# lmb-freiburg/optical-flow-2d-data-generation

Measured on AMD Instinct MI355X. Metric: training samples/sec (img0+img1+flow, 512x384), higher is better.
Workload: dtype u8 blends / fp64 affines -> f32 planes

## Files before the change

### optical-flow-2d-data-generation_amd/csrc/kernels.hip

```cpp
#include <hip/hip_runtime.h>
#include <stdint.h>
#include <type_traits>

#include "../../include/ofdg_detmath.h"
#include "ofdg_device.h"
#include "warpfields.h"

namespace ofdg {

__device__ __forceinline__ int iround_d(double v) {
  return (int)((v < 0.0) ? v - 0.5 : v + 0.5);
}
__device__ __forceinline__ void xform(const Mat& m, double& x, double& y) {
  double t = x;
  x = t * m.sx + y * m.shx + m.tx;
  y = t * m.shy + y * m.sy + m.ty;
}
__device__ __forceinline__ long long floordiv64(long long a, long long b) {
  long long q = (long long)floor((double)a / (double)b);
  long long r = a - q * b;
  if (r < 0) --q;
  else if (r >= b) ++q;
  return q;
}
// ... 497 lines not shown
  int nonzero = 0;
  for (int r = 0; r < rows; ++r) {
    const int2 cv = *reinterpret_cast<const int2*>(&tc.cover[r][c2]);
    const int2 ar = *reinterpret_cast<const int2*>(&tc.area[r][c2]);
    const int s2 = cv.x + cv.y;
    const int base = tc.carry[r] + wave_scan_incl(s2) - s2;
    int a0 = ((base + cv.x) << 9) - ar.x, a1 = ((base + s2) << 9) - ar.y;
    a0 >>= 9; a1 >>= 9;
    a0 = a0 < 0 ? -a0 : a0; a1 = a1 < 0 ? -a1 : a1;
    a0 = a0 > 255 ? 255 : a0; a1 = a1 > 255 ? 255 : a1;
    if (in_range) { *reinterpret_cast<uint16_t*>(dst + (size_t)r * W + c2) = (uint16_t)(a0 | (a1 << 8)); nonzero |= a0 | a1; }
  }
  const unsigned long long nz = __ballot(nonzero != 0);
  if (blockmask) {
    const int half = lane >> 5;
    if ((lane & 31) == 0 && ((nz >> (32 * half)) & 0xFFFFFFFFull)) {
      const int nbx = (W + kTileW - 1) / kTileW, nby = (H + kBandRows - 1) / kBandRows;
      atomicOr(blockmask + ((size_t)(sample * nby + band) * nbx + (X0 / kTileW + half)) * 2 + (sf & 1), 1ull << obj_local);
    }
  }
  __builtin_amdgcn_fence(__ATOMIC_ACQ_REL, "workgroup");
}

__global__ __launch_bounds__(64 * kRasterWaves) void raster_kernel(const DevShapeFrame* __restrict__ frames,
                                                     const int4* __restrict__ items,
                                                     const int* __restrict__ item_count,
                                                     const int2* __restrict__ verts, int W, int H,
                                                     uint8_t* __restrict__ cov,
                                                     unsigned long long* __restrict__ blockmask_next, int n_mask_words,
                                                     unsigned long long* __restrict__ blockmask) {
  __shared__ __attribute__((aligned(16))) RasterWs s_ws[kRasterWaves];
  step_kernel_priority();
  const int wave = threadIdx.x >> 6, lane = threadIdx.x & 63;
  for (int gid = blockIdx.x * blockDim.x + threadIdx.x; gid < n_mask_words; gid += gridDim.x * blockDim.x) blockmask_next[gid] = 0ull;
  const int n_items = *item_count;
  const int n_waves = gridDim.x * kRasterWaves;
  typedef OFDG_CONSTANT const int4 ConstItem;
  typedef OFDG_CONSTANT const DevShapeFrame ConstFrame;
  int it = __builtin_amdgcn_readfirstlane(blockIdx.x * kRasterWaves + wave);
  if (it >= n_items) return;
  struct Item { int sf, band, X0, X1; };
  struct Frame { int nv, x0, y0, x1, y1, sample, obj_local; };
  auto item_at = [&](int i) {
    const int4 q = ((ConstItem*)items)[i];
    return Item{q.x, q.y, q.z, q.w};
  };
  auto frame_of = [&](int sf) {
    const ConstFrame& f = ((ConstFrame*)frames)[sf];
    return Frame{f.n_verts, f.x0, f.y0, f.x1, f.y1, f.pad[0], f.pad[1]};
  };
  auto uni = [](int x) { return __builtin_amdgcn_readfirstlane(x); };
  int it1 = it + n_waves;
  Item I0 = item_at(it), I1 = item_at(it1 < n_items ? it1 : it);
  Frame F0 = frame_of(I0.sf);
  int2 pa = verts[(size_t)I0.sf * kMaxVerts + lane], pb = verts[(size_t)I0.sf * kMaxVerts + lane + 1];
  for (;;) {
    I0 = Item{uni(I0.sf), uni(I0.band), uni(I0.X0), uni(I0.X1)};
    I1 = Item{uni(I1.sf), uni(I1.band), uni(I1.X0), uni(I1.X1)};
    F0 = Frame{uni(F0.nv), uni(F0.x0), uni(F0.y0), uni(F0.x1), uni(F0.y1), uni(F0.sample), uni(F0.obj_local)};
    it1 = uni(it1);
    const int it2 = it1 + n_waves;
    const Item I2 = item_at(it2 < n_items ? it2 : it1 < n_items ? it1 : it);
    const Frame F1 = frame_of(I1.sf);
    const int2 na = verts[(size_t)I1.sf * kMaxVerts + lane], nb = verts[(size_t)I1.sf * kMaxVerts + lane + 1];
    raster_item(s_ws[wave], verts + (size_t)I0.sf * kMaxVerts, F0.nv, F0.x0, F0.y0, F0.x1, F0.y1, I0.sf, I0.band, I0.X0, I0.X1, W, H, cov, blockmask,
                F0.sample, F0.obj_local, lane, pa, pb);
    if (it1 >= n_items) break;
    I0 = I1; F0 = F1; I1 = I2; pa = na; pb = nb;
    it = it1; it1 = it2;
  }
}

__device__ __forceinline__ int aa_byte(int c) { return c == 255 ? 255 : (255 * c) >> 8; }
__device__ __forceinline__ int div255(int a) { return (a + 1 + (a >> 8)) >> 8; }
__device__ __forceinline__ int blend(int d, int s, int m) { return div255(m * s + (255 - m) * d); }

__device__ __forceinline__ uint32_t blend_px(uint32_t d, uint32_t s, uint32_t m) {
  const uint32_t im = 255u - m;
  uint32_t rb = m * (s & 0x00FF00FFu) + im * (d & 0x00FF00FFu);
  uint32_t g = m * ((s >> 8) & 255u) + im * ((d >> 8) & 255u);
  rb = ((rb + 0x00010001u + ((rb >> 8) & 0x00FF00FFu)) >> 8) & 0x00FF00FFu;
  g = (g + 1u + (g >> 8)) >> 8;
  return rb | (g << 8);
}

__device__ __forceinline__ float byte_over_255(int u) {
  const float fu = (float)u, c = 0x1.010102p-8f;
  const float q0 = __fmul_rn(fu, c);
  return __fmaf_rn(__fmaf_rn(-q0, 255.f, fu), c, q0);
}
__device__ __forceinline__ int comp_add(int u, int v) {
  const float fu = byte_over_255(u), fv = byte_over_255(v);
  const float t = __fmul_rn(__fsub_rn(1.f, fu), __fsub_rn(1.f, fv));
// ... 1257 lines not shown
#pragma unroll
    for (int c = 0; c < 3; ++c) {
      const double v1 = u32_to_double((t0 >> (8 * c)) & 255u), v2 = u32_to_double((t1 >> (8 * c)) & 255u);
      out |= (uint32_t)(unsigned char)(al1 * v1 + al * v2) << (8 * c);
    }
    return out;
  }
  if (sdim == n) return t0;
  const uint32_t d0 = u1, d1 = u2, d2 = (uint32_t)n - u1 - u2;
  uint32_t acc[3];
#pragma unroll
  for (int c = 0; c < 3; ++c)
    acc[c] = __umul24((t2 >> (8 * c)) & 255u, d2) + (__umul24((t1 >> (8 * c)) & 255u, d1) + __umul24((t0 >> (8 * c)) & 255u, d0));
  if (div24) return mulhi_u24(acc[0], mdiv) | (mulhi_u24(acc[1], mdiv) << 8) | (mulhi_u24(acc[2], mdiv) << 16);
  uint32_t out = 0;
#pragma unroll
  for (int c = 0; c < 3; ++c) {
    uint32_t q = __umulhi(acc[c], mdiv);
    q -= (q * (uint32_t)n > acc[c]) ? 1u : 0u;
    out |= q << (8 * c);
  }
  return out;
}
__global__ __launch_bounds__(64) void bgprep_stream_kernel(const DevBgPrep* __restrict__ prep, DevResizeTabs T, int W, int H, int n_samples,
                                                           int cap_cw, int cap_ch, uint32_t* __restrict__ B, uint32_t* __restrict__ err,
                                                           uint32_t* __restrict__ paths) {
  __shared__ uint32_t s_c[kPrepG][kPrepCW];
  extern __shared__ int s_first[];
  const int TW = 2 * W, TH = 2 * H, lane = threadIdx.x;
  {
    int running = 0;
    if (lane == 0) s_first[0] = 0;
    for (int c = 0; c < n_samples; c += 64) {
      const int i = c + lane;
      int nt = 0;
      if (i < n_samples) {
        const DevBgPrep& q = prep[i];
        const bool fits = prep_sample_fits(q, cap_cw, cap_ch);
        if (!fits && blockIdx.x == 0) atomicOr(err, kErrBgPrepCapacity);
        nt = fits ? prep_tile_cols(q) * prep_tile_rows(q) : 0;
      }
      const int incl = wave_scan_incl(nt);
      if (i < n_samples) s_first[i + 1] = running + incl;
      running += __shfl(incl, 63, 64);
    }
  }
  __syncthreads();
  const int total = __builtin_amdgcn_readfirstlane(s_first[n_samples]);
  auto sample_of = [&](int t) {
    int n = 0;
    for (int c = 0; c < n_samples; c += 64) {
      const int i = c + lane;
      n += __popcll(__ballot(i < n_samples && t >= s_first[i + 1]));
    }
    return __builtin_amdgcn_readfirstlane(n);
  };
  auto tab_index = [](int n, int dim, int k) { return (uint32_t)(n < dim ? n * dim + k : 0); };
  struct PrepBox { int cw, ch, rx0, ry0, rx1, ry1; };
  typedef OFDG_CONSTANT const DevBgPrep ConstPrep;
  auto box_fields = [&](int s) { const ConstPrep& q = ((ConstPrep*)prep)[s]; return PrepBox{q.cw, q.ch, q.rx0, q.ry0, q.rx1, q.ry1}; };
  auto box_of = [&](const PrepBox& q, int t, int s, PrepTile& F) {
    const int tcols = (q.rx1 - q.rx0 + kPrepW) / kPrepW;
    const int ti = t - __builtin_amdgcn_readfirstlane(s_first[s]), ty = ti / tcols, tx = ti - ty * tcols;
    F.s = s;
    F.bx0 = q.rx0 + tx * kPrepW; F.bx1 = min(F.bx0 + kPrepW - 1, q.rx1);
    F.by0 = q.ry0 + ty * kPrepH; F.by1 = min(F.by0 + kPrepH - 1, q.ry1);
  };
  int t = blockIdx.x;
  if (t < (int)(gridDim.x / (8 * kPrepRun)) * (8 * kPrepRun)) {
    const int xcd = t & 7, slot = t >> 3;
    t = ((slot / kPrepRun) * 8 + xcd) * kPrepRun + (slot % kPrepRun);
  }
  if (t >= total) return;
  PrepTile cur;
  int ex0, ex1, ey0, ey1;
  {
    const int s0 = sample_of(t);
    const PrepBox q = box_fields(s0);
    box_of(q, t, s0, cur);
    ex0 = tab_entry_uniform(T.at_x, tab_index(q.cw, TW, cur.bx0)); ex1 = tab_entry_uniform(T.at_x, tab_index(q.cw, TW, cur.bx1));
    ey0 = tab_entry_uniform(T.at_y, tab_index(q.ch, TH, cur.by0)); ey1 = tab_entry_uniform(T.at_y, tab_index(q.ch, TH, cur.by1));
  }
  for (;;) {
    const int tn = t + (int)gridDim.x;
    const bool more = tn < total;
    const int sc = __builtin_amdgcn_readfirstlane(cur.s);
    const int sn = more ? sample_of(tn) : sc;
    const DevBgPrep p = ((ConstPrep*)prep)[sc];
    const PrepBox qn = box_fields(sn);
    prep_finish_tile(p, cur, TW, TH, ex0, ex1, ey0, ey1);
    const int bx0 = cur.bx0, bx1 = cur.bx1, by0 = cur.by0, by1 = cur.by1;
    const int cx0 = cur.cx0, cx1 = cur.cx1, cy0 = cur.cy0, cy1 = cur.cy1;
    const int ncw = cx1 - cx0 + 1, nch = cy1 - cy0 + 1;
    const int x = bx0 + lane;
    const bool have_x = x <= bx1;
    const AxisEntry ex = axis_entry(p.cw, TW, min(x, bx1), T.at_x, T.alpha_x);
    const AxisEntry ey = axis_entry(p.ch, TH, min(by0 + lane, by1), T.at_y, T.alpha_y);
    PrepTile nxt = cur;
    int nx0 = 0, nx1 = 0, ny0 = 0, ny1 = 0;
    if (more) {
      box_of(qn, tn, sn, nxt);
      nx0 = tab_entry_uniform(T.at_x, tab_index(qn.cw, TW, nxt.bx0)); nx1 = tab_entry_uniform(T.at_x, tab_index(qn.cw, TW, nxt.bx1));
      ny0 = tab_entry_uniform(T.at_y, tab_index(qn.ch, TH, nxt.by0)); ny1 = tab_entry_uniform(T.at_y, tab_index(qn.ch, TH, nxt.by1));
    }
    if (!cur.fits) {
      if (lane == 0) atomicOr(err, kErrBgPrepCapacity);
    } else {
// ... 109 lines not shown
        } else {
        int xg = x, cwg = p.cw, chg = p.ch;
        asm volatile("" : "+v"(xg), "+s"(cwg), "+s"(chg));
        for (int r = 0; r < rows; ++r) {
          const int j = cy0 + g0 + r;
          m0 = m1; m1 = m2;
          m2 = have_x ? axis_texel(cwg, TW, xg, ex.u1, ex.u2, x_exact, s_c[r][xi0], s_c[r][xi1], s_c[r][xi2], xdiv, xdiv24, T.alpha_x) : 0u;
          emit_rows(j, [&](int dj, uint32_t v1, uint32_t v2) {
            uint32_t t0 = m2, t1 = m2;
            if (dj >= 2) { t0 = m0; t1 = m1; } else if (dj == 1) { t0 = m1; }
            return axis_texel(chg, TH, y, v1, v2, (v2 >> 31) != 0u, t0, t1, m2, ydiv, ydiv24, T.alpha_y);
          });
        }
        }
        __syncthreads();
      }
    }
    if (!more) break;
    ex0 = nx0; ex1 = nx1; ey0 = ny0; ey1 = ny1;
    cur = nxt;
    t = tn;
  }
}

__global__ __launch_bounds__(256) void bgprep_kernel(const DevBgPrep* __restrict__ prep, int W, int H, uint32_t* __restrict__ bgtex) {
  const int TW = 2 * W, TH = 2 * H, quads = TW / 4;
  const int s = blockIdx.y;
  const int i = blockIdx.x * blockDim.x + threadIdx.x;
  if (i >= quads * TH) return;
  const int v = i / quads, u0 = (i - v * quads) * 4;
  const DevBgPrep p = prep[s];
  if (v < p.ry0 || v > p.ry1 || u0 + 3 < p.rx0 || u0 > p.rx1) return;
  uint4 o;
  o.x = bgprep_texel(p, u0, v);
  o.y = bgprep_texel(p, u0 + 1, v);
  o.z = bgprep_texel(p, u0 + 2, v);
  o.w = bgprep_texel(p, u0 + 3, v);
  *reinterpret_cast<uint4*>(bgtex + (size_t)s * TW * TH + (size_t)v * TW + u0) = o;
}

__global__ __launch_bounds__(256) void pool_synth_kernel(uint32_t* __restrict__ pool, int n, int w, int h, uint32_t seed) {
  const size_t total = (size_t)n * w * h;
  for (size_t i = (size_t)blockIdx.x * blockDim.x + threadIdx.x; i < total; i += (size_t)gridDim.x * blockDim.x) {
    const uint32_t tex = (uint32_t)(i / ((size_t)w * h));
    const uint32_t rem = (uint32_t)(i - (size_t)tex * w * h);
    const uint32_t y = rem / w, x = rem - y * w;
// ... 115 lines not shown
```

### optical-flow-2d-data-generation_amd/csrc/ofdg_api.hip

```cpp
#include <hip/hip_runtime.h>
#include <hip/hip_ext.h>

#include <algorithm>
#include <cmath>
#include <cstdio>
#include <cstdlib>
#include <cstring>
#include <memory>
#include <string>
#include <vector>

#include "../../include/ofdg.h"
#include "kernels.hip"
#include "sampler_counter.hip"
#include "ofdg_device.h"
#include "realize.h"
#include "sampler_ref.h"
#include "warpfields.h"

using namespace ofdg;

static thread_local std::string g_create_error;
static const int g_hw_queues_env = [] { const char* q = std::getenv("GPU_MAX_HW_QUEUES"); return q ? std::atoi(q) : 0; }();

// ... 34 lines not shown
  std::vector<std::pair<int, int>> mixed_sizes;
  std::vector<uint32_t*> mixed_images;
  std::vector<DevTexEntry> tex_table;
  DevTexEntry* d_tex_table = nullptr;
  int pool_kind = OFDG_POOL_UNIFORM;
  uint32_t pool_seed = 0;
  std::unique_ptr<RefSampler> sampler;
  long long step = 0;
  struct Slot {
    RealizedBatch batch;
    DevBuf<DevShape> d_shapes;
    DevBuf<DevShapeFrame> d_frames;
    DevBuf<int2> d_verts;
    DevBuf<DevObject> d_objects;
    DevBuf<DevSample> d_samples;
    DevBuf<char> d_rec;
    DevBuf<int4> d_items;
    DevBuf<DevBgPrep> d_bgprep;
    DevBuf<uint32_t> d_bgtex;
    DevBuf<uint32_t> d_bgC;
    DevBuf<unsigned long long> d_blockmask;
    int res_objects = 0;
    bool bgprep_pending = false;
    int box_parity = 0;
    size_t box_stride = 0;
    int mask_used[2] = {0, 0};
    hipEvent_t ev_uploaded = nullptr;
    bool upload_pending = false;
    hipStream_t upload_stream = nullptr;
    DevBuf<DevCropRef> d_croptab;
    DevBuf<float> d_bgwarp;
    DevBuf<unsigned> d_bgwarp_max;
    hipEvent_t compose_event = nullptr;
    bool compose_pending = false;
    hipStream_t compose_stream = nullptr;
    int* d_item_count = nullptr;
    int res_samples = 0, res_shapes = 0;
  };
  static constexpr int kUserSlots = 16;
  Slot slots[kUserSlots];
  struct Stage {
    void* h = nullptr;
    size_t bytes = 0;
    hipEvent_t free_ev = nullptr;
    bool pending = false;
  };
// ... 673 lines not shown
  return OFDG_OK;
}
static void bgprep_caps(ofdg_ctx* c, int* cap_cw, int* cap_ch, bool* fusable) {
  if (c->bg_cap_n == c->pool_n && c->bg_cap_cw > 0) { *cap_cw = c->bg_cap_cw; *cap_ch = c->bg_cap_ch; *fusable = c->bg_fusable; return; }
  const int TW = 2 * c->prm.width, TH = 2 * c->prm.height;
  int cw = (int)((float)TW / 0.75f) + 2, ch = (int)((float)TH / 0.75f) + 2;
  bool all_large = true;
  auto small = [&](int w, int h) { if (w < TW || h < TH) { all_large = false; cw = std::max(cw, w + h / 8 + 4); ch = std::max(ch, h + w / 8 + 4); } };
  if (c->pool_mixed) for (const auto& wh : c->mixed_sizes) small(wh.first, wh.second);
  else small(c->pool_w, c->pool_h);
  c->bg_cap_cw = cw; c->bg_cap_ch = ch; c->bg_cap_n = c->pool_n; c->bg_fusable = all_large;
  *cap_cw = cw; *cap_ch = ch; *fusable = all_large;
}

static int reserve_workspaces(ofdg_ctx* c, size_t n_shapes) {
  const size_t need_cov = n_shapes * 2 * (size_t)c->prm.width * c->prm.height + 16;
  if (need_cov <= c->chains[0].cov.cap) return OFDG_OK;
  HIP_OK(c, hipDeviceSynchronize());
  for (int k = 0; k < c->n_chains; ++k) HIP_OK(c, c->chains[k].cov.reserve(need_cov));
  return OFDG_OK;
}

static int prepare_backgrounds(ofdg_ctx* c, ofdg_ctx::Slot& sl, int n, bool records_resident, hipStream_t s, uint32_t* err, hipEvent_t stop = nullptr);
static int launch_counter_sampler(ofdg_ctx* c, ofdg_ctx::Slot& sl, long long first_index, hipStream_t s, uint32_t* err) {
  const int stride = sl.res_shapes / sl.res_samples;
  const int prep = c->prm.background_prep ? 1 : 0;
  CsRealizeDims D{c->prm.width, c->prm.height, c->pool_n, c->pool_w, c->pool_h, sl.res_samples, stride, prep,
                  c->prm.mode == 9 ? c->crop_server.n_crops : 0, c->fg_src.stride, c->fg_src.origin, c->bg_src.stride, c->bg_src.origin,
                  (unsigned long long)(uintptr_t)c->pool, c->d_tex_table, c->prm.mode == 9 ? c->d_cs_croptab : nullptr};
  hipLaunchKernelGGL(cs_sample_realize_kernel, dim3(sl.res_samples * kCsGroups), dim3(64), 0, s, c->cs_mode, D, first_index,
                     sl.d_shapes.p, sl.d_objects.p, sl.d_samples.p, err, sl.d_bgprep.p);
  HIP_OK(c, hipGetLastError());
  sl.bgprep_pending = prep != 0;
  return OFDG_OK;
}

static void* own_stream(ofdg_ctx* c, void* stream) { return stream == OFDG_STREAM_OWN ? ofdg_stream(c) : stream; }

static ofdg_ctx::Chain& take_chain(ofdg_ctx* c) {
  const int k = (int)(c->next_chain % (unsigned)c->n_chains);
  c->next_chain++;
  c->last_chain = k;
  return c->chains[k];
}
static hipStream_t chain_stream(const ofdg_ctx* c, const ofdg_ctx::Chain& ch, hipStream_t st) { return c->overlap ? ch.stream : st; }

// ... 8 lines not shown
  return OFDG_OK;
}
static int discard_all_prepared(ofdg_ctx* c) {
  c->bg_cap_n = -1;
  for (int k = 0; k < c->n_chains; ++k) { int rc = discard_prepared(c, c->chains[k]); if (rc != OFDG_OK) return rc; }
  return OFDG_OK;
}

static RenderDims render_dims(const ofdg_ctx* c, const ofdg_ctx::Slot& sl) {
  const int W = c->prm.width, H = c->prm.height;
  RenderDims dm;
  dm.W = W; dm.H = H; dm.pool_w = c->pool_w; dm.pool_h = c->pool_h;
  dm.use_aa = c->prm.use_antialiasing ? 1 : 0;
  dm.n_samples = sl.res_samples;
  dm.n_shapes = sl.res_shapes;
  dm.tiles_x = (W + kTileW - 1) / kTileW;
  dm.tiles_y = (H + kTileH - 1) / kTileH;
  dm.bg_pitch = c->prm.background_prep ? 2 * W : c->bg_src.pitch;
  dm.fg_pitch = c->fg_src.pitch;
  return dm;
}

static int launch_prepare(ofdg_ctx* c, ofdg_ctx::Chain& ch, ofdg_ctx::Slot& sl, hipStream_t st, long long cs_first_index = -1,
                          bool hand_over = true) {
  const int W = c->prm.width, H = c->prm.height;
  const int n_sf = sl.res_shapes * 2;
  const RenderDims dm = render_dims(c, sl);
  { int rc = discard_prepared(c, ch); if (rc != OFDG_OK) return rc; }
  const long long ticket = c->ticket++;
  uint32_t* const err = err_word(c, ticket);
  hipEvent_t* ev = nullptr;
  if (c->profiling && c->ev_sets > 0 && (c->launch_count % c->ev_stride) == 0) {
    const size_t set = (size_t)(c->ev_alloc++ % c->ev_sets);
    ev = &c->ev[set * 6];
    c->ev_composed[set] = 0;
    c->ev_bgprep[set] = 0;
  }
  c->launch_count++;
  if (!c->overlap) {
    if (c->have_last_user_st && c->last_user_st != st) HIP_OK(c, hipDeviceSynchronize());
    c->last_user_st = st; c->have_last_user_st = true;
  }
  hipStream_t S = chain_stream(c, ch, st);
  uint8_t* cov = ch.cov.p;
  if (sl.upload_pending && sl.upload_stream != S) {
    if (hipEventQuery(sl.ev_uploaded) == hipSuccess) sl.upload_pending = false;
    else HIP_OK(c, hipStreamWaitEvent(S, sl.ev_uploaded, 0));
  }
  if (ch.done_pending && ch.done_stream != S) {
    if (hipEventQuery(ch.ev_done) != hipSuccess) HIP_OK(c, hipStreamWaitEvent(S, ch.ev_done, 0));
    ch.done_pending = false;
  }
  if (sl.compose_pending && sl.compose_stream != S) {
    if (hipEventQuery(sl.compose_event) == hipSuccess) sl.compose_pending = false;
    else HIP_OK(c, hipStreamWaitEvent(S, sl.compose_event, 0));
  }
  const DevCropRef* croptab = cs_first_index >= 0 ? c->d_cs_croptab : sl.d_croptab.p;
  HIP_OK(c, take_err_word(c, ticket, S));
  if (cs_first_index >= 0) {
    int rc = launch_counter_sampler(c, sl, cs_first_index, S, err);
    if (rc != OFDG_OK) return rc;
  }
  const int bp = sl.box_parity;
  sl.box_parity ^= 1;
  unsigned long long* box_cur = sl.d_blockmask.p + (size_t)bp * sl.box_stride;
  unsigned long long* box_next = sl.d_blockmask.p + (size_t)(bp ^ 1) * sl.box_stride;
  sl.mask_used[bp] = sl.res_samples * dm.tiles_x * ((H + kBandRows - 1) / kBandRows) * 2;
  const int n_mask_words = sl.mask_used[bp ^ 1];
  const bool prof_prep = ev && c->profiling == 2;
  hipExtLaunchKernelGGL(geom_kernel, dim3(std::max(1, (n_sf + kGeomWaves - 1) / kGeomWaves)), dim3(64 * kGeomWaves), 0, S,
                        prof_prep ? ev[0] : nullptr, prof_prep ? ev[1] : nullptr, 0, sl.d_shapes.p, sl.res_shapes, c->d_cs_tab, W, H,
                        sl.d_frames.p, sl.d_verts.p, box_cur, err, sl.d_item_count, sl.d_items.p, croptab);
  HIP_OK(c, hipGetLastError());
  const bool prep_last = sl.bgprep_pending;
  hipEvent_t last_stop = ev ? (c->profiling == 2 ? nullptr : ev[4]) : (hand_over ? ch.ev_prep : nullptr);
  hipExtLaunchKernelGGL(raster_kernel, dim3(kRasterGrid * 4 / kRasterWaves), dim3(64 * kRasterWaves), 0, S, nullptr,
                        (ev && (c->profiling == 2 || prep_last)) ? ev[3] : (prep_last ? nullptr : last_stop), 0,
                        sl.d_frames.p, sl.d_items.p, sl.d_item_count, sl.d_verts.p, W, H, cov, box_next, n_mask_words, box_cur);
  HIP_OK(c, hipGetLastError());
  if (prep_last) {
    int rcb = prepare_backgrounds(c, sl, sl.res_samples, true, S, err, (ev && c->profiling == 2) ? ev[2] : last_stop);
    if (rcb != OFDG_OK) return rcb;
    sl.bgprep_pending = false;
    if (ev) c->ev_bgprep[(size_t)(ev - c->ev.data()) / 6] = 1;
  }
  if (ev && hand_over) HIP_OK(c, hipEventRecord(ch.ev_prep, S));
  ch.prep.valid = true; ch.prep.slot = &sl; ch.prep.first_index = cs_first_index; ch.prep.n = sl.res_samples;
  ch.prep.box_cur = box_cur; ch.prep.croptab = croptab; ch.prep.ev = ev; ch.prep.stream = S; ch.prep.ticket = ticket;
  ch.prep.ahead = false;
  return OFDG_OK;
}

static int launch_compose(ofdg_ctx* c, ofdg_ctx::Chain& ch, float* d_img0, float* d_img1, float* d_flow, hipStream_t st) {
  if (!ch.prep.valid) { c->err = "internal: compose without a prepared batch"; return OFDG_EINVAL; }
  ofdg_ctx::Slot& sl = *ch.prep.slot;
  const int W = c->prm.width, H = c->prm.height;
  const RenderDims dm = render_dims(c, sl);
  const int compose_grid = dm.tiles_x * dm.tiles_y * dm.n_samples * 4;
  hipEvent_t* ev = ch.prep.ev;
  unsigned long long* box_cur = ch.prep.box_cur;
  const DevCropRef* croptab = ch.prep.croptab;
  uint8_t* cov = ch.cov.p;
  const hipStream_t S = ch.prep.stream;
  const bool foreign = S != st;
  const uint32_t* bgpool = c->prm.background_prep ? sl.d_bgtex.p : (c->pool_bg ? c->pool_bg : c->pool);
  const uint32_t* fgpool = c->pool_fg ? c->pool_fg : c->pool;
  if (c->prm.background_prep && !bgpool) { c->err = "background_prep: the slot has no prepared backgrounds"; return OFDG_EINVAL; }
// ... 30 lines not shown
    const bool span_is_the_launch = c->profiling == 2 || (!foreign && !ch.prep.ahead);
    if (span_is_the_launch) {
      c->ev_count++;
      c->ev_composed[(size_t)(ev - c->ev.data()) / 6] = 1;
    }
  }
  if (done) {
    sl.compose_pending = true; sl.compose_stream = CS; sl.compose_event = done;
    ch.done_pending = true; ch.done_stream = CS;
  } else {
    sl.compose_pending = false;
  }
  return OFDG_OK;
}

static int launch_resident(ofdg_ctx* c, ofdg_ctx::Chain& ch, ofdg_ctx::Slot& sl, float* d_img0, float* d_img1, float* d_flow,
                           hipStream_t st, long long cs_first_index = -1) {
  int rc = launch_prepare(c, ch, sl, st, cs_first_index, chain_stream(c, ch, st) != st);
  if (rc != OFDG_OK) return rc;
  return launch_compose(c, ch, d_img0, d_img1, d_flow, st);
}

constexpr int kPrepGrid = 4096;
static int ensure_bgprep_tables(ofdg_ctx* c) {
  const int TW = 2 * c->prm.width, TH = 2 * c->prm.height;
  if (c->bg_tab_w == TW && c->bg_tab_h == TH) return OFDG_OK;
  auto build = [&](int s, DevBuf<uint16_t>& d_at, DevBuf<double>& d_alpha) -> int {
    std::vector<uint16_t> at((size_t)s * s, 0);
    std::vector<double> alpha((size_t)s * s, 0.0);
    for (int n = 1; n < s; ++n) {
      const double f = s > 1 ? (n - 1.) / (s - 1) : 0;
      double curr = 0, old = 0;
      int pos = 0;
      for (int x = 0; x < s; ++x) {
        alpha[(size_t)n * s + x] = curr - (unsigned int)curr;
        at[(size_t)n * s + x] = (uint16_t)pos;
        old = curr;
        curr = std::min(n - 1., curr + f);
        pos += (int)((unsigned int)curr - (unsigned int)old);
      }
    }
    HIP_OK(c, d_at.reserve(at.size()));
    HIP_OK(c, d_alpha.reserve(alpha.size()));
    HIP_OK(c, hipMemcpy(d_at.p, at.data(), at.size() * sizeof(uint16_t), hipMemcpyHostToDevice));
    HIP_OK(c, hipMemcpy(d_alpha.p, alpha.data(), alpha.size() * sizeof(double), hipMemcpyHostToDevice));
    return OFDG_OK;
  };
  if (TW > 65535 || TH > 65535) { c->err = "background_prep: frame too large for the resize tables"; return OFDG_EINVAL; }
  HIP_OK(c, hipDeviceSynchronize());
  int rc = build(TW, c->d_bg_at_x, c->d_bg_alpha_x);
  if (rc == OFDG_OK) rc = build(TH, c->d_bg_at_y, c->d_bg_alpha_y);
  if (rc != OFDG_OK) return rc;
  c->bg_tab_w = TW; c->bg_tab_h = TH;
  return OFDG_OK;
}

static int prepare_backgrounds(ofdg_ctx* c, ofdg_ctx::Slot& sl, int n, bool records_resident, hipStream_t s, uint32_t* err, hipEvent_t stop) {
  const int W = c->prm.width, H = c->prm.height;
  if (!records_resident || !sl.d_bgprep.p || sl.d_bgprep.cap < (size_t)n) { c->err = "internal: background preparation without its records"; return OFDG_EINVAL; }
  HIP_OK(c, sl.d_bgtex.reserve((size_t)n * 4 * W * H));
  int cap_cw, cap_ch;
  bool fusable;
  bgprep_caps(c, &cap_cw, &cap_ch, &fusable);
  const bool staged = c->prm.background_prep == 1;
  constexpr int kBgPrepBlocks = 192;
  if (staged) {
    int rct = ensure_bgprep_tables(c);
    if (rct != OFDG_OK) return rct;
  }
  if (!staged) {
    hipExtLaunchKernelGGL(bgprep_kernel, dim3((W * H + 255) / 256, n), dim3(256), 0, s, nullptr, stop, 0, sl.d_bgprep.p, W, H, sl.d_bgtex.p);
    HIP_OK(c, hipGetLastError());
    return OFDG_OK;
  }
  const DevResizeTabs T{c->d_bg_at_x.p, c->d_bg_alpha_x.p, c->d_bg_at_y.p, c->d_bg_alpha_y.p};
  if (fusable && n <= kPrepMaxSamples) {
    hipExtLaunchKernelGGL(bgprep_stream_kernel, dim3(kPrepGrid), dim3(64), (size_t)(n + 1) * sizeof(int), s, nullptr, stop, 0, sl.d_bgprep.p, T, W, H, n, cap_cw, cap_ch, sl.d_bgtex.p, err,
                          c->d_prep_paths);
    HIP_OK(c, hipGetLastError());
    return OFDG_OK;
  }
  HIP_OK(c, sl.d_bgC.reserve((size_t)n * cap_cw * cap_ch));
  hipLaunchKernelGGL(bgprep_rotcrop_kernel, dim3(kBgPrepBlocks, n), dim3(256), 0, s, sl.d_bgprep.p, T, W, H, cap_cw, cap_ch, sl.d_bgC.p,
                     err);
  hipExtLaunchKernelGGL(bgprep_resize_kernel, dim3(kBgPrepBlocks, n), dim3(256), 0, s, nullptr, stop, 0, sl.d_bgprep.p, T, W, H, cap_cw, cap_ch, sl.d_bgC.p,
                        sl.d_bgtex.p);
  HIP_OK(c, hipGetLastError());
  return OFDG_OK;
}

static int upload_slot(ofdg_ctx* c, ofdg_ctx::Slot& sl, const ofdg_task* tasks, int n_tasks, const ofdg_blueprint* bps,
                       int n_bps, hipStream_t st, ofdg_ctx::Stage& stage, bool shared) {
  if (!c->pool && !c->pool_mixed) { c->err = "Could not open texture collection (no texture pool)"; return OFDG_ETEXTURES; }
  { int rcf = finalise_pool(c); if (rcf != OFDG_OK) return rcf; }
  { int rct = ensure_tex_table(c); if (rct != OFDG_OK) return rct; }
  RealizeConfig cfg{c->prm.width, c->prm.height, c->prm.mode, c->pool_n, c->pool_w, c->pool_h, c->prm.background_prep};
  cfg.pool_addr = (uint64_t)(uintptr_t)c->pool;
  cfg.tex_table = c->pool_mixed && c->prm.background_prep ? c->tex_table.data() : nullptr;
  cfg.fg_stride = c->fg_src.stride; cfg.fg_origin = c->fg_src.origin; cfg.bg_stride = c->bg_src.stride; cfg.bg_origin = c->bg_src.origin;
  if (stage.pending) {
    if (hipEventQuery(stage.free_ev) != hipSuccess) HIP_OK(c, hipEventSynchronize(stage.free_ev));
    stage.pending = false;
  }
  if (sl.compose_pending && sl.compose_stream != st) {
    HIP_OK(c, hipStreamWaitEvent(st, sl.compose_event, 0));
    sl.compose_pending = false;
  }
  sl.res_samples = 0;
  int rc = realize_batch(cfg, tasks, n_tasks, bps, n_bps, &sl.batch, &c->err, &c->crop_server);
  if (rc != OFDG_OK) return rc;
// ... 151 lines not shown
  if (c->prm.background_prep) {
    HIP_OK(c, sl.d_bgprep.reserve(n));
    HIP_OK(c, sl.d_bgtex.reserve((size_t)n * 4 * W * H));
  }
  if (!sl.d_item_count) {
    HIP_OK(c, hipMalloc((void**)&sl.d_item_count, sizeof(int)));
    HIP_OK(c, hipMemset(sl.d_item_count, 0, sizeof(int)));
    HIP_OK(c, hipDeviceSynchronize());
  }
  sl.res_samples = n;
  sl.res_shapes = (int)shapes_cap;
  sl.res_objects = (int)n_obj;
  sl.batch.samples.clear();
  return OFDG_OK;
}

int ofdg_forward_counter(ofdg_ctx* c, long long first_index, int n_samples, float* d_img0, float* d_img1, float* d_flow,
                         void* stream) {
  if (!c || !d_img0 || !d_img1 || !d_flow || first_index < 0) return OFDG_EINVAL;
  stream = own_stream(c, stream);
  const int k = (int)(c->next_chain % (unsigned)c->n_chains);
  ofdg_ctx::Chain& ch = take_chain(c);
  hipStream_t st = (hipStream_t)stream;
  auto prepare_on = [&](ofdg_ctx::Chain& cj, long long first, hipStream_t s_, bool hand_over) -> int {
    if (cj.prep.valid && cj.prep.slot == &cj.slot && cj.prep.first_index == first && cj.prep.n == n_samples) return OFDG_OK;
    int rc = prepare_counter_slot(c, cj.slot, n_samples);
    if (rc != OFDG_OK) return rc;
    return launch_prepare(c, cj, cj.slot, s_, first, hand_over);
  };
  int rc = prepare_on(ch, first_index, st, chain_stream(c, ch, st) != st);
  if (rc != OFDG_OK) return rc;
  rc = launch_compose(c, ch, d_img0, d_img1, d_flow, st);
  if (rc != OFDG_OK) return rc;
  const long long prev_first = c->last_first;
  c->last_first = first_index;
  if (c->overlap && c->lookahead > 0) {
    const long long stride = (prev_first >= 0 && first_index > prev_first) ? first_index - prev_first
                                                                             : (long long)n_samples * std::max(1, c->prm.world_size);
    for (int d = 1; d <= std::min(c->lookahead, c->n_chains - 1); ++d) {
      ofdg_ctx::Chain& cj = c->chains[(k + d) % c->n_chains];
      if (prepare_on(cj, first_index + (long long)d * stride, cj.stream, true) != OFDG_OK) { (void)discard_prepared(c, cj); break; }
      cj.prep.ahead = true;
    }
  }
  return OFDG_OK;
}

int ofdg_num_chains(const ofdg_ctx* c) { return c ? c->n_chains : OFDG_EINVAL; }
void* ofdg_stream(ofdg_ctx* c) {
  if (!c) return nullptr;
  return (void*)c->chains[c->next_chain % (unsigned)c->n_chains].stream;
}

int ofdg_sample_counter(ofdg_ctx* c, long long first_index, int n_samples, ofdg_task* tasks, ofdg_blueprint* bps) {
  if (!c || !tasks || !bps || n_samples < 1 || first_index < 0) return OFDG_EINVAL;
  HIP_OK(c, hipDeviceSynchronize());
  HIP_OK(c, c->d_cs_bps.reserve((size_t)n_samples * kCsBlueprintsPerSample));
  HIP_OK(c, c->d_cs_nobj.reserve(n_samples));
  hipLaunchKernelGGL(cs_sample_kernel, dim3(n_samples * kCsGroups), dim3(64), 0, 0, c->cs_mode, first_index, n_samples,
                     c->prm.mode == 9 ? c->crop_server.n_crops : 0, c->d_cs_bps.p,
                     c->d_cs_nobj.p);
  HIP_OK(c, hipGetLastError());
  std::vector<int> nobj(n_samples);
  HIP_OK(c, hipMemcpy(bps, c->d_cs_bps.p, (size_t)n_samples * kCsBlueprintsPerSample * sizeof(ofdg_blueprint), hipMemcpyDeviceToHost));
// ... 347 lines not shown
  const size_t sf = (size_t)(s.first_shape + shape) * 2 + frame;
  HIP_OK(c, hipDeviceSynchronize());
  DevShapeFrame f;
  HIP_OK(c, hipMemcpy(&f, sl.d_frames.p + sf, sizeof(f), hipMemcpyDeviceToHost));
  std::vector<uint8_t> tmp((size_t)W * H);
  HIP_OK(c, hipMemcpy(tmp.data(), c->chains[c->last_chain].cov.p + sf * W * H, tmp.size(), hipMemcpyDeviceToHost));
  std::memset(coverage_host, 0, tmp.size());
  for (int y = f.y0; y <= f.y1; ++y)
    for (int x = f.x0; x <= f.x1; ++x) coverage_host[(size_t)y * W + x] = tmp[(size_t)y * W + x];
  return OFDG_OK;
}

int ofdg_debug_item_count(ofdg_ctx* c) {
  if (!c || !c->last_slot || !c->last_slot->d_item_count) return OFDG_EINVAL;
  int n = 0;
  if (hipDeviceSynchronize() != hipSuccess) return OFDG_EHIP;
  if (hipMemcpy(&n, c->last_slot->d_item_count, sizeof(int), hipMemcpyDeviceToHost) != hipSuccess) return OFDG_EHIP;
  return n;
}

int ofdg_debug_bgprep_tiles(ofdg_ctx* c, int* tiles, int* workgroups) {
  if (!c || !tiles || !workgroups || !c->last_slot) return OFDG_EINVAL;
  const ofdg_ctx::Slot& sl = *c->last_slot;
  *tiles = 0; *workgroups = kPrepGrid;
  int cap_cw, cap_ch;
  bool fusable;
  bgprep_caps(c, &cap_cw, &cap_ch, &fusable);
  const int n = sl.res_samples;
  if (c->prm.background_prep != 1 || !fusable || n > kPrepMaxSamples || n < 1 || !sl.d_bgprep.p) return OFDG_OK;
  HIP_OK(c, hipDeviceSynchronize());
  std::vector<DevBgPrep> rec((size_t)n);
  HIP_OK(c, hipMemcpy(rec.data(), sl.d_bgprep.p, rec.size() * sizeof(DevBgPrep), hipMemcpyDeviceToHost));
  for (const DevBgPrep& q : rec)
    if (prep_sample_fits(q, cap_cw, cap_ch)) *tiles += prep_tile_cols(q) * prep_tile_rows(q);
  return OFDG_OK;
}

int ofdg_debug_bgprep_paths(ofdg_ctx* c, unsigned* counts9) {
  if (!c || !counts9) return OFDG_EINVAL;
  HIP_OK(c, hipDeviceSynchronize());
  if (!c->d_prep_paths) {
    HIP_OK(c, hipMalloc((void**)&c->d_prep_paths, 9 * sizeof(uint32_t)));
    HIP_OK(c, hipMemset(c->d_prep_paths, 0, 9 * sizeof(uint32_t)));
  }
  HIP_OK(c, hipMemcpy(counts9, c->d_prep_paths, 9 * sizeof(uint32_t), hipMemcpyDeviceToHost));
  HIP_OK(c, hipMemset(c->d_prep_paths, 0, 9 * sizeof(uint32_t)));
  return OFDG_OK;
// ... 20 lines not shown

int ofdg_kernel_ms(ofdg_ctx* c, const char* kernel, float* ms) {
  if (!c || !kernel || !ms) return OFDG_EINVAL;
  int i = -1;
  if (!std::strcmp(kernel, "geom")) i = 0;
  else if (!std::strcmp(kernel, "raster")) i = 1;
  else if (!std::strcmp(kernel, "compose")) i = 2;
  else if (!std::strcmp(kernel, "background_prep")) i = 3;
  if (i < 0) { c->err = "unknown kernel name"; return OFDG_EINVAL; }
  if (!c->profiling || c->ev_count == 0 || (i < 2 && c->profiling != 2)) {
    c->err = "no profiled launch of that kernel yet (ofdg_set_profiling)";
    return OFDG_EINVAL;
  }
  int n = 0;
  double acc = 0;
  for (int k = 0; k < c->ev_sets; ++k) {
    if (!c->ev_composed[(size_t)k]) continue;
    if (i == 3 && !c->ev_bgprep[(size_t)k]) continue;
    ++n;
    hipEvent_t* ev = &c->ev[(size_t)k * 6];
    HIP_OK(c, hipEventSynchronize(ev[5]));
    float t = 0;
    if (i == 3) {
      HIP_OK(c, hipEventElapsedTime(&t, ev[3], ev[c->profiling == 2 ? 2 : 4]));
      acc += t;
      continue;
    }
    HIP_OK(c, hipEventElapsedTime(&t, ev[i == 0 ? 0 : (i == 2 ? 4 : 1)], ev[2 * i + 1]));
    acc += t;
  }
  if (n == 0) { c->err = "no profiled launch of that kernel yet (ofdg_set_profiling)"; return OFDG_EINVAL; }
  *ms = (float)(acc / n);
  return OFDG_OK;
}

int ofdg_debug_tables(ofdg_ctx* c, uint8_t* add_tbl, uint8_t* sub_tbl, uint8_t* aa_tbl, uint8_t* blend_tbl, int s_fixed) {
  if (!c) return OFDG_EINVAL;
  uint8_t* d = nullptr;
  HIP_OK(c, hipMalloc((void**)&d, 3 * 65536 + 256));
  hipLaunchKernelGGL(tables_kernel, dim3(256), dim3(256), 0, 0, d, d + 65536, d + 3 * 65536, d + 2 * 65536, s_fixed);
  HIP_OK(c, hipGetLastError());
  HIP_OK(c, hipMemcpy(add_tbl, d, 65536, hipMemcpyDeviceToHost));
  HIP_OK(c, hipMemcpy(sub_tbl, d + 65536, 65536, hipMemcpyDeviceToHost));
  HIP_OK(c, hipMemcpy(blend_tbl, d + 2 * 65536, 65536, hipMemcpyDeviceToHost));
  HIP_OK(c, hipMemcpy(aa_tbl, d + 3 * 65536, 256, hipMemcpyDeviceToHost));
  HIP_OK(c, hipFree(d));
  return OFDG_OK;
// ... 24 lines not shown
```

Measured before the change: 345,800.

## Fuse raster and background-prep kernels into one role-split launch

Measured after the change: 345,200, median of 3. No clear change (-0.2%).

```diff
diff --git a/optical-flow-2d-data-generation_amd/csrc/kernels.hip b/optical-flow-2d-data-generation_amd/csrc/kernels.hip
--- a/optical-flow-2d-data-generation_amd/csrc/kernels.hip
+++ b/optical-flow-2d-data-generation_amd/csrc/kernels.hip
@@ -543,22 +543,18 @@
   __builtin_amdgcn_fence(__ATOMIC_ACQ_REL, "workgroup");
 }
 
-__global__ __launch_bounds__(64 * kRasterWaves) void raster_kernel(const DevShapeFrame* __restrict__ frames,
-                                                     const int4* __restrict__ items,
-                                                     const int* __restrict__ item_count,
-                                                     const int2* __restrict__ verts, int W, int H,
-                                                     uint8_t* __restrict__ cov,
-                                                     unsigned long long* __restrict__ blockmask_next, int n_mask_words,
-                                                     unsigned long long* __restrict__ blockmask) {
-  __shared__ __attribute__((aligned(16))) RasterWs s_ws[kRasterWaves];
-  step_kernel_priority();
+__device__ __forceinline__ void raster_role(RasterWs* s_ws, int wg, int n_wg, const DevShapeFrame* __restrict__ frames,
+                                            const int4* __restrict__ items, const int* __restrict__ item_count,
+                                            const int2* __restrict__ verts, int W, int H, uint8_t* __restrict__ cov,
+                                            unsigned long long* __restrict__ blockmask_next, int n_mask_words,
+                                            unsigned long long* __restrict__ blockmask) {
   const int wave = threadIdx.x >> 6, lane = threadIdx.x & 63;
-  for (int gid = blockIdx.x * blockDim.x + threadIdx.x; gid < n_mask_words; gid += gridDim.x * blockDim.x) blockmask_next[gid] = 0ull;
+  for (int gid = wg * (64 * kRasterWaves) + threadIdx.x; gid < n_mask_words; gid += n_wg * (64 * kRasterWaves)) blockmask_next[gid] = 0ull;
   const int n_items = *item_count;
-  const int n_waves = gridDim.x * kRasterWaves;
+  const int n_waves = n_wg * kRasterWaves;
   typedef OFDG_CONSTANT const int4 ConstItem;
   typedef OFDG_CONSTANT const DevShapeFrame ConstFrame;
-  int it = __builtin_amdgcn_readfirstlane(blockIdx.x * kRasterWaves + wave);
+  int it = __builtin_amdgcn_readfirstlane(wg * kRasterWaves + wave);
   if (it >= n_items) return;
   struct Item { int sf, band, X0, X1; };
   struct Frame { int nv, x0, y0, x1, y1, sample, obj_local; };
@@ -590,6 +586,18 @@
     I0 = I1; F0 = F1; I1 = I2; pa = na; pb = nb;
     it = it1; it1 = it2;
   }
+}
+
+__global__ __launch_bounds__(64 * kRasterWaves) void raster_kernel(const DevShapeFrame* __restrict__ frames,
+                                                     const int4* __restrict__ items,
+                                                     const int* __restrict__ item_count,
+                                                     const int2* __restrict__ verts, int W, int H,
+                                                     uint8_t* __restrict__ cov,
+                                                     unsigned long long* __restrict__ blockmask_next, int n_mask_words,
+                                                     unsigned long long* __restrict__ blockmask) {
+  __shared__ __attribute__((aligned(16))) RasterWs s_ws[kRasterWaves];
+  step_kernel_priority();
+  raster_role(s_ws, blockIdx.x, gridDim.x, frames, items, item_count, verts, W, H, cov, blockmask_next, n_mask_words, blockmask);
 }
 
 __device__ __forceinline__ int aa_byte(int c) { return c == 255 ? 255 : (255 * c) >> 8; }
@@ -1893,11 +1901,10 @@
   }
   return out;
 }
-__global__ __launch_bounds__(64) void bgprep_stream_kernel(const DevBgPrep* __restrict__ prep, DevResizeTabs T, int W, int H, int n_samples,
-                                                           int cap_cw, int cap_ch, uint32_t* __restrict__ B, uint32_t* __restrict__ err,
-                                                           uint32_t* __restrict__ paths) {
-  __shared__ uint32_t s_c[kPrepG][kPrepCW];
-  extern __shared__ int s_first[];
+__device__ __forceinline__ void bgprep_role(uint32_t (&s_c)[kPrepG][kPrepCW], int* s_first, int wg, int n_wg,
+                                            const DevBgPrep* __restrict__ prep, DevResizeTabs T, int W, int H, int n_samples,
+                                            int cap_cw, int cap_ch, uint32_t* __restrict__ B, uint32_t* __restrict__ err,
+                                            uint32_t* __restrict__ paths) {
   const int TW = 2 * W, TH = 2 * H, lane = threadIdx.x;
   {
     int running = 0;
@@ -1908,7 +1915,7 @@
       if (i < n_samples) {
         const DevBgPrep& q = prep[i];
         const bool fits = prep_sample_fits(q, cap_cw, cap_ch);
-        if (!fits && blockIdx.x == 0) atomicOr(err, kErrBgPrepCapacity);
+        if (!fits && wg == 0) atomicOr(err, kErrBgPrepCapacity);
         nt = fits ? prep_tile_cols(q) * prep_tile_rows(q) : 0;
       }
       const int incl = wave_scan_incl(nt);
@@ -1937,8 +1944,8 @@
     F.bx0 = q.rx0 + tx * kPrepW; F.bx1 = min(F.bx0 + kPrepW - 1, q.rx1);
     F.by0 = q.ry0 + ty * kPrepH; F.by1 = min(F.by0 + kPrepH - 1, q.ry1);
   };
-  int t = blockIdx.x;
-  if (t < (int)(gridDim.x / (8 * kPrepRun)) * (8 * kPrepRun)) {
+  int t = wg;
+  if (t < (n_wg / (8 * kPrepRun)) * (8 * kPrepRun)) {
     const int xcd = t & 7, slot = t >> 3;
     t = ((slot / kPrepRun) * 8 + xcd) * kPrepRun + (slot % kPrepRun);
   }
@@ -1953,7 +1960,7 @@
     ey0 = tab_entry_uniform(T.at_y, tab_index(q.ch, TH, cur.by0)); ey1 = tab_entry_uniform(T.at_y, tab_index(q.ch, TH, cur.by1));
   }
   for (;;) {
-    const int tn = t + (int)gridDim.x;
+    const int tn = t + n_wg;
     const bool more = tn < total;
     const int sc = __builtin_amdgcn_readfirstlane(cur.s);
     const int sn = more ? sample_of(tn) : sc;
@@ -2109,6 +2116,37 @@
     t = tn;
   }
 }
+__global__ __launch_bounds__(64) void bgprep_stream_kernel(const DevBgPrep* __restrict__ prep, DevResizeTabs T, int W, int H, int n_samples,
+                                                           int cap_cw, int cap_ch, uint32_t* __restrict__ B, uint32_t* __restrict__ err,
+                                                           uint32_t* __restrict__ paths) {
+  __shared__ uint32_t s_c[kPrepG][kPrepCW];
+  extern __shared__ int s_first[];
+  bgprep_role(s_c, s_first, blockIdx.x, gridDim.x, prep, T, W, H, n_samples, cap_cw, cap_ch, B, err, paths);
+}
+
+union RasterFusedLds {
+  RasterWs ws;
+  uint32_t c[kPrepG][kPrepCW];
+};
+__global__ __launch_bounds__(64) void raster_bgprep_kernel(const DevShapeFrame* __restrict__ frames, const int4* __restrict__ items,
+                                                           const int* __restrict__ item_count, const int2* __restrict__ verts, int W, int H,
+                                                           uint8_t* __restrict__ cov, unsigned long long* __restrict__ blockmask_next,
+                                                           int n_mask_words, unsigned long long* __restrict__ blockmask, int n_raster,
+                                                           const DevBgPrep* __restrict__ prep, DevResizeTabs T, int n_samples, int cap_cw,
+                                                           int cap_ch, uint32_t* __restrict__ B, uint32_t* __restrict__ err,
+                                                           uint32_t* __restrict__ paths) {
+  static_assert(kRasterWaves == 1, "one wave per workgroup in either role");
+  extern __shared__ __attribute__((aligned(16))) char s_dyn[];
+  RasterFusedLds& u = *reinterpret_cast<RasterFusedLds*>(s_dyn);
+  const int wg = blockIdx.x;
+  if (wg < n_raster) {
+    step_kernel_priority();
+    raster_role(&u.ws, wg, n_raster, frames, items, item_count, verts, W, H, cov, blockmask_next, n_mask_words, blockmask);
+  } else {
+    bgprep_role(u.c, reinterpret_cast<int*>(s_dyn + sizeof(RasterFusedLds)), wg - n_raster, (int)gridDim.x - n_raster, prep, T, W, H,
+                n_samples, cap_cw, cap_ch, B, err, paths);
+  }
+}
 
 __global__ __launch_bounds__(256) void bgprep_kernel(const DevBgPrep* __restrict__ prep, int W, int H, uint32_t* __restrict__ bgtex) {
   const int TW = 2 * W, TH = 2 * H, quads = TW / 4;
diff --git a/optical-flow-2d-data-generation_amd/csrc/ofdg_api.hip b/optical-flow-2d-data-generation_amd/csrc/ofdg_api.hip
--- a/optical-flow-2d-data-generation_amd/csrc/ofdg_api.hip
+++ b/optical-flow-2d-data-generation_amd/csrc/ofdg_api.hip
@@ -80,6 +80,7 @@
     DevBuf<unsigned long long> d_blockmask;
     int res_objects = 0;
     bool bgprep_pending = false;
+    int bgprep_groups = 0;
     int box_parity = 0;
     size_t box_stride = 0;
     int mask_used[2] = {0, 0};
@@ -799,6 +800,12 @@
 }
 
 static int prepare_backgrounds(ofdg_ctx* c, ofdg_ctx::Slot& sl, int n, bool records_resident, hipStream_t s, uint32_t* err, hipEvent_t stop = nullptr);
+static bool bgprep_one_launch(ofdg_ctx* c, int n);
+struct RasterArgs {
+  const DevShapeFrame* frames; const int4* items; const int* item_count; const int2* verts;
+  uint8_t* cov; unsigned long long* box_next; int n_mask_words; unsigned long long* box_cur;
+};
+static int launch_raster_bgprep(ofdg_ctx* c, ofdg_ctx::Slot& sl, const RasterArgs& ra, hipStream_t s, uint32_t* err, hipEvent_t stop);
 static int launch_counter_sampler(ofdg_ctx* c, ofdg_ctx::Slot& sl, long long first_index, hipStream_t s, uint32_t* err) {
   const int stride = sl.res_shapes / sl.res_samples;
   const int prep = c->prm.background_prep ? 1 : 0;
@@ -853,7 +860,7 @@
 }
 
 static int launch_prepare(ofdg_ctx* c, ofdg_ctx::Chain& ch, ofdg_ctx::Slot& sl, hipStream_t st, long long cs_first_index = -1,
-                          bool hand_over = true) {
+                          bool hand_over = true, bool fuse = true) {
   const int W = c->prm.width, H = c->prm.height;
   const int n_sf = sl.res_shapes * 2;
   const RenderDims dm = render_dims(c, sl);
@@ -899,21 +906,30 @@
   sl.mask_used[bp] = sl.res_samples * dm.tiles_x * ((H + kBandRows - 1) / kBandRows) * 2;
   const int n_mask_words = sl.mask_used[bp ^ 1];
   const bool prof_prep = ev && c->profiling == 2;
+  const bool prep_last = sl.bgprep_pending;
+  const bool fused = prep_last && fuse && bgprep_one_launch(c, sl.res_samples);
   hipExtLaunchKernelGGL(geom_kernel, dim3(std::max(1, (n_sf + kGeomWaves - 1) / kGeomWaves)), dim3(64 * kGeomWaves), 0, S,
-                        prof_prep ? ev[0] : nullptr, prof_prep ? ev[1] : nullptr, 0, sl.d_shapes.p, sl.res_shapes, c->d_cs_tab, W, H,
+                        prof_prep ? ev[0] : nullptr, (prof_prep || (ev && fused)) ? ev[1] : nullptr, 0, sl.d_shapes.p, sl.res_shapes, c->d_cs_tab, W, H,
                         sl.d_frames.p, sl.d_verts.p, box_cur, err, sl.d_item_count, sl.d_items.p, croptab);
   HIP_OK(c, hipGetLastError());
-  const bool prep_last = sl.bgprep_pending;
   hipEvent_t last_stop = ev ? (c->profiling == 2 ? nullptr : ev[4]) : (hand_over ? ch.ev_prep : nullptr);
-  hipExtLaunchKernelGGL(raster_kernel, dim3(kRasterGrid * 4 / kRasterWaves), dim3(64 * kRasterWaves), 0, S, nullptr,
-                        (ev && (c->profiling == 2 || prep_last)) ? ev[3] : (prep_last ? nullptr : last_stop), 0,
-                        sl.d_frames.p, sl.d_items.p, sl.d_item_count, sl.d_verts.p, W, H, cov, box_next, n_mask_words, box_cur);
-  HIP_OK(c, hipGetLastError());
-  if (prep_last) {
-    int rcb = prepare_backgrounds(c, sl, sl.res_samples, true, S, err, (ev && c->profiling == 2) ? ev[2] : last_stop);
+  if (fused) {
+    const RasterArgs ra{sl.d_frames.p, sl.d_items.p, sl.d_item_count, sl.d_verts.p, cov, box_next, n_mask_words, box_cur};
+    int rcb = launch_raster_bgprep(c, sl, ra, S, err, (ev && c->profiling == 2) ? ev[3] : last_stop);
     if (rcb != OFDG_OK) return rcb;
     sl.bgprep_pending = false;
-    if (ev) c->ev_bgprep[(size_t)(ev - c->ev.data()) / 6] = 1;
+    if (ev) c->ev_bgprep[(size_t)(ev - c->ev.data()) / 6] = 2;
+  } else {
+    hipExtLaunchKernelGGL(raster_kernel, dim3(kRasterGrid * 4 / kRasterWaves), dim3(64 * kRasterWaves), 0, S, nullptr,
+                          (ev && (c->profiling == 2 || prep_last)) ? ev[3] : (prep_last ? nullptr : last_stop), 0,
+                          sl.d_frames.p, sl.d_items.p, sl.d_item_count, sl.d_verts.p, W, H, cov, box_next, n_mask_words, box_cur);
+    HIP_OK(c, hipGetLastError());
+    if (prep_last) {
+      int rcb = prepare_backgrounds(c, sl, sl.res_samples, true, S, err, (ev && c->profiling == 2) ? ev[2] : last_stop);
+      if (rcb != OFDG_OK) return rcb;
+      sl.bgprep_pending = false;
+      if (ev) c->ev_bgprep[(size_t)(ev - c->ev.data()) / 6] = 1;
+    }
   }
   if (ev && hand_over) HIP_OK(c, hipEventRecord(ch.ev_prep, S));
   ch.prep.valid = true; ch.prep.slot = &sl; ch.prep.first_index = cs_first_index; ch.prep.n = sl.res_samples;
@@ -990,6 +1006,9 @@
 }
 
 constexpr int kPrepGrid = 4096;
+constexpr int kFusedRaster = kRasterGrid * 4 / kRasterWaves;
+constexpr int kFusedPrep = kPrepGrid;
+static_assert(kFusedRaster % 8 == 0, "the preparation's workgroups keep their XCDs");
 static int ensure_bgprep_tables(ofdg_ctx* c) {
   const int TW = 2 * c->prm.width, TH = 2 * c->prm.height;
   if (c->bg_tab_w == TW && c->bg_tab_h == TH) return OFDG_OK;
@@ -1023,19 +1042,27 @@
   return OFDG_OK;
 }
 
-static int prepare_backgrounds(ofdg_ctx* c, ofdg_ctx::Slot& sl, int n, bool records_resident, hipStream_t s, uint32_t* err, hipEvent_t stop) {
+static bool bgprep_one_launch(ofdg_ctx* c, int n) {
+  int cap_cw, cap_ch;
+  bool fusable;
+  bgprep_caps(c, &cap_cw, &cap_ch, &fusable);
+  return c->prm.background_prep == 1 && fusable && n <= kPrepMaxSamples;
+}
+static int bgprep_setup(ofdg_ctx* c, ofdg_ctx::Slot& sl, int n, bool records_resident, int* cap_cw, int* cap_ch, bool* fusable) {
   const int W = c->prm.width, H = c->prm.height;
   if (!records_resident || !sl.d_bgprep.p || sl.d_bgprep.cap < (size_t)n) { c->err = "internal: background preparation without its records"; return OFDG_EINVAL; }
   HIP_OK(c, sl.d_bgtex.reserve((size_t)n * 4 * W * H));
+  bgprep_caps(c, cap_cw, cap_ch, fusable);
+  if (c->prm.background_prep == 1) return ensure_bgprep_tables(c);
+  return OFDG_OK;
+}
+static int prepare_backgrounds(ofdg_ctx* c, ofdg_ctx::Slot& sl, int n, bool records_resident, hipStream_t s, uint32_t* err, hipEvent_t stop) {
+  const int W = c->prm.width, H = c->prm.height;
   int cap_cw, cap_ch;
   bool fusable;
-  bgprep_caps(c, &cap_cw, &cap_ch, &fusable);
+  { int rcs = bgprep_setup(c, sl, n, records_resident, &cap_cw, &cap_ch, &fusable); if (rcs != OFDG_OK) return rcs; }
   const bool staged = c->prm.background_prep == 1;
   constexpr int kBgPrepBlocks = 192;
-  if (staged) {
-    int rct = ensure_bgprep_tables(c);
-    if (rct != OFDG_OK) return rct;
-  }
   if (!staged) {
     hipExtLaunchKernelGGL(bgprep_kernel, dim3((W * H + 255) / 256, n), dim3(256), 0, s, nullptr, stop, 0, sl.d_bgprep.p, W, H, sl.d_bgtex.p);
     HIP_OK(c, hipGetLastError());
@@ -1046,6 +1073,7 @@
     hipExtLaunchKernelGGL(bgprep_stream_kernel, dim3(kPrepGrid), dim3(64), (size_t)(n + 1) * sizeof(int), s, nullptr, stop, 0, sl.d_bgprep.p, T, W, H, n, cap_cw, cap_ch, sl.d_bgtex.p, err,
                           c->d_prep_paths);
     HIP_OK(c, hipGetLastError());
+    sl.bgprep_groups = kPrepGrid;
     return OFDG_OK;
   }
   HIP_OK(c, sl.d_bgC.reserve((size_t)n * cap_cw * cap_ch));
@@ -1054,6 +1082,21 @@
   hipExtLaunchKernelGGL(bgprep_resize_kernel, dim3(kBgPrepBlocks, n), dim3(256), 0, s, nullptr, stop, 0, sl.d_bgprep.p, T, W, H, cap_cw, cap_ch, sl.d_bgC.p,
                         sl.d_bgtex.p);
   HIP_OK(c, hipGetLastError());
+  return OFDG_OK;
+}
+
+static int launch_raster_bgprep(ofdg_ctx* c, ofdg_ctx::Slot& sl, const RasterArgs& ra, hipStream_t s, uint32_t* err, hipEvent_t stop) {
+  const int W = c->prm.width, H = c->prm.height, n = sl.res_samples;
+  int cap_cw, cap_ch;
+  bool fusable;
+  { int rcs = bgprep_setup(c, sl, n, true, &cap_cw, &cap_ch, &fusable); if (rcs != OFDG_OK) return rcs; }
+  const DevResizeTabs T{c->d_bg_at_x.p, c->d_bg_alpha_x.p, c->d_bg_at_y.p, c->d_bg_alpha_y.p};
+  hipExtLaunchKernelGGL(raster_bgprep_kernel, dim3(kFusedRaster + kFusedPrep), dim3(64), sizeof(RasterFusedLds) + (size_t)(n + 1) * sizeof(int), s,
+                        nullptr, stop, 0,
+                        ra.frames, ra.items, ra.item_count, ra.verts, W, H, ra.cov, ra.box_next, ra.n_mask_words, ra.box_cur, kFusedRaster,
+                        sl.d_bgprep.p, T, n, cap_cw, cap_ch, sl.d_bgtex.p, err, c->d_prep_paths);
+  HIP_OK(c, hipGetLastError());
+  sl.bgprep_groups = kFusedPrep;
   return OFDG_OK;
 }
 
@@ -1251,13 +1294,13 @@
   const int k = (int)(c->next_chain % (unsigned)c->n_chains);
   ofdg_ctx::Chain& ch = take_chain(c);
   hipStream_t st = (hipStream_t)stream;
-  auto prepare_on = [&](ofdg_ctx::Chain& cj, long long first, hipStream_t s_, bool hand_over) -> int {
+  auto prepare_on = [&](ofdg_ctx::Chain& cj, long long first, hipStream_t s_, bool hand_over, bool ahead) -> int {
     if (cj.prep.valid && cj.prep.slot == &cj.slot && cj.prep.first_index == first && cj.prep.n == n_samples) return OFDG_OK;
     int rc = prepare_counter_slot(c, cj.slot, n_samples);
     if (rc != OFDG_OK) return rc;
-    return launch_prepare(c, cj, cj.slot, s_, first, hand_over);
+    return launch_prepare(c, cj, cj.slot, s_, first, hand_over, !ahead);
   };
-  int rc = prepare_on(ch, first_index, st, chain_stream(c, ch, st) != st);
+  int rc = prepare_on(ch, first_index, st, chain_stream(c, ch, st) != st, false);
   if (rc != OFDG_OK) return rc;
   rc = launch_compose(c, ch, d_img0, d_img1, d_flow, st);
   if (rc != OFDG_OK) return rc;
@@ -1268,7 +1311,7 @@
                                                                              : (long long)n_samples * std::max(1, c->prm.world_size);
     for (int d = 1; d <= std::min(c->lookahead, c->n_chains - 1); ++d) {
       ofdg_ctx::Chain& cj = c->chains[(k + d) % c->n_chains];
-      if (prepare_on(cj, first_index + (long long)d * stride, cj.stream, true) != OFDG_OK) { (void)discard_prepared(c, cj); break; }
+      if (prepare_on(cj, first_index + (long long)d * stride, cj.stream, true, true) != OFDG_OK) { (void)discard_prepared(c, cj); break; }
       cj.prep.ahead = true;
     }
   }
@@ -1662,7 +1705,7 @@
 int ofdg_debug_bgprep_tiles(ofdg_ctx* c, int* tiles, int* workgroups) {
   if (!c || !tiles || !workgroups || !c->last_slot) return OFDG_EINVAL;
   const ofdg_ctx::Slot& sl = *c->last_slot;
-  *tiles = 0; *workgroups = kPrepGrid;
+  *tiles = 0; *workgroups = sl.bgprep_groups ? sl.bgprep_groups : kPrepGrid;
   int cap_cw, cap_ch;
   bool fusable;
   bgprep_caps(c, &cap_cw, &cap_ch, &fusable);
@@ -1729,7 +1772,8 @@
     HIP_OK(c, hipEventSynchronize(ev[5]));
     float t = 0;
     if (i == 3) {
-      HIP_OK(c, hipEventElapsedTime(&t, ev[3], ev[c->profiling == 2 ? 2 : 4]));
+      if (c->ev_bgprep[(size_t)k] == 2) HIP_OK(c, hipEventElapsedTime(&t, ev[1], ev[c->profiling == 2 ? 3 : 4]));
+      else HIP_OK(c, hipEventElapsedTime(&t, ev[3], ev[c->profiling == 2 ? 2 : 4]));
       acc += t;
       continue;
     }
```
